# modelstreaming/ams

Measured on AMD Instinct MI355X. Metric: frames/sec student infer (DeeplabV3+MobileNetV2, 512x1024) + distill-steps/sec, higher is better.
Workload: dtype f32 (2xfp16 split products)

## Files before the change

ams_amd/csrc/k_pw_f16.hip:

```cpp
#include <type_traits>

#include "pw_common.hpp"
#include "split_bf16.hpp"

namespace ams {

__global__ void split_w_f16_kernel(const float* __restrict__ w, int64_t sk, int64_t sn, int K, int N, int Kp, unsigned short* __restrict__ hi,
                                   unsigned short* __restrict__ lo) {
    const int64_t i = blockIdx.x * (int64_t)blockDim.x + threadIdx.x;
    if (i >= (int64_t)N * Kp) return;
    const int n = (int)(i / Kp), k = (int)(i % Kp);
    const float v = k < K ? w[k * sk + n * sn] : 0.f;
    unsigned short h, l;
    split1_f16(v, h, l);
    hi[i] = h;
    lo[i] = l;
}

int launch_split_weights_f16(const float* w, int64_t sk, int64_t sn, int K, int N, int Kp, uint16_t* hi, uint16_t* lo, hipStream_t st) {
    const int64_t n = (int64_t)N * Kp;
    hipLaunchKernelGGL(split_w_f16_kernel, dim3(cdiv(n, 256)), dim3(256), 0, st, w, sk, sn, K, N, Kp, hi, lo);
    AMS_CHECK_LAUNCH();
    return AMS_OK;
}

__global__ void pack_h2i_kernel(const float* __restrict__ x, int64_t n8, u32x4* __restrict__ out) {
    const int64_t i = blockIdx.x * (int64_t)blockDim.x + threadIdx.x;
    if (i >= n8) return;
    const float4 u = ld4(x + 8 * i), v = ld4(x + 8 * i + 4);
    f16x8 h, l;
    split8_f16(u, v, h, l);
    out[2 * i] = __builtin_bit_cast(u32x4, h);
    out[2 * i + 1] = __builtin_bit_cast(u32x4, l);
}

int launch_pack_h2i(const float* x, int64_t M, int C, float* out, hipStream_t st) {
    AMS_REQUIRE(C % 8 == 0 && M > 0, "pack_h2i: C (%d) must be a multiple of 8", C);
    const int64_t n8 = M * (C / 8);
    hipLaunchKernelGGL(pack_h2i_kernel, dim3((unsigned)cdiv64(n8, 256)), dim3(256), 0, st, x, n8, reinterpret_cast<u32x4*>(out));
    AMS_CHECK_LAUNCH();
    return AMS_OK;
}

__device__ __forceinline__ f32x4 mma_f16(const u32x4& a, const u32x4& b, const f32x4& c) {
    return __builtin_amdgcn_mfma_f32_16x16x32_f16(__builtin_bit_cast(f16x8, a), __builtin_bit_cast(f16x8, b), c, 0, 0, 0);
}

constexpr int pwh_waves(int rm, int nt, int nw) { return nw >= 9 ? 3 : nw == 8 ? 2 : rm * nt > 12 ? 1 : rm * nt > 6 ? 2 : 3; }
constexpr int pwh_epw(int nw, int slab) { return nw * slab <= 60 * 1024 ? nw : nw % 5 == 0 && 5 * slab <= 60 * 1024 ? 5 : nw % 4 == 0 ? 4 : nw % 3 == 0 ? 3 : 1; }
constexpr bool pwh_dyn(int nw, int epi) { return nw >= 9 && epi != EPI_GENERIC; }

template <int RM, int NT, int EPI, int XP, int NW = 4, int D = 2, int ABL = 0, int XF = 0>
__global__ __launch_bounds__(64 * NW, pwh_waves(RM, NT, NW)) void pw_gemm_f16x3_l(PwArgs a, const unsigned short* __restrict__ w0, int64_t plane, int Kp,
                                                                                  int n_tiles_n, unsigned nblocks, unsigned n_full) {
    constexpr int NP = 2, NTH = 64 * NW;
    constexpr int PITCH = 32;
    constexpr int ROWS = 16 * NT;
    constexpr int NPIECE = NP * ROWS * 4;
    constexpr int NREG = (NPIECE + NTH - 1) / NTH;
    constexpr int SLAB = 16 * (16 * NT + 4) * 4;
    constexpr bool DYN = pwh_dyn(NW, EPI);
    constexpr int EPW = (EPI == EPI_GENERIC || DYN) ? NW : pwh_epw(NW, SLAB);
    static_assert(NW % EPW == 0, "epilogue rounds");
    static_assert(XF == 0 || (XP == 0 && EPI == EPI_PLAIN), "the operand transform runs on f32 operands with the plain epilogue");
    constexpr int W_BYTES = 2 * NP * ROWS * PITCH * 2, OUT_BYTES = EPI == EPI_GENERIC ? 16 : EPW * SLAB + (EPI == EPI_PLAIN && NW == 4 ? 4 * 16 * NT * 4 : 0);
    __shared__ __attribute__((aligned(16))) unsigned char smem_static[DYN ? 16 : (W_BYTES > OUT_BYTES ? W_BYTES : OUT_BYTES)];
    extern __shared__ __attribute__((aligned(16))) unsigned char smem_dyn[];
    unsigned char* smem = DYN ? smem_dyn : smem_static;
    typedef unsigned short (*WStage)[NP][ROWS * PITCH];
    WStage sW = reinterpret_cast<WStage>(smem);
    float* sOutAll = reinterpret_cast<float*>(smem);
    __shared__ __attribute__((aligned(16))) float sSc[16 * NT], sSh[16 * NT];
    constexpr int XVS = XF != 0 ? 1024 : 4;
    __shared__ __attribute__((aligned(16))) float sXv[XF == 1 ? 2 * XVS : 4];
    const bool half = blockIdx.x >= n_full;
    const unsigned lb = half ? xcd_remap(blockIdx.x - n_full, nblocks - n_full) : xcd_remap(blockIdx.x, n_full);
    const int tile_n = lb % n_tiles_n;
    const int64_t tile_m = lb / n_tiles_n;
    const int tid = threadIdx.x, wave = tid >> 6, lane = tid & 63, l15 = lane & 15, q = lane >> 4;
    const int n0 = tile_n * ROWS;
    const int nrg = half ? RM / 2 : RM;
    const int64_t m_base = half ? (int64_t)(n_full / n_tiles_n) * (16 * NW * RM) + tile_m * (8 * NW * RM) + wave * (8 * RM)
                                : tile_m * (16 * NW * RM) + wave * (16 * RM);
    const int K = a.K, n_stages = Kp / 32;
    const int n_iter = (n_stages + D - 1) / D * D;

    u32x4 wring[D][NREG];
    const unsigned short* wsrc[NREG];
    int wdst[NREG];
#pragma unroll
    for (int u = 0; u < NREG; ++u) {
        const int e = tid + u * NTH < NPIECE ? tid + u * NTH : NPIECE - 1;
        const int which = e / (ROWS * 4), r = e - which * (ROWS * 4), n = r >> 2, part = r & 3;
        int nn = n0 + n;
        if (nn > a.N - 1) nn = a.N - 1;
        wsrc[u] = w0 + which * plane + (int64_t)nn * Kp + part * 8;
        wdst[u] = which * (ROWS * PITCH) + n * PITCH + (part ^ (((n >> 3) & 1) << 1)) * 8;
    }
    auto load_stage = [&](int s, u32x4 (&wreg)[NREG]) {
        if (s > n_stages - 1) s = n_stages - 1;
#pragma unroll
        for (int u = 0; u < NREG; ++u) wreg[u] = *reinterpret_cast<const u32x4*>(wsrc[u] + s * 32);
    };
    auto store_stage = [&](int buf, const u32x4 (&wreg)[NREG]) {
        unsigned short* base = &sW[buf][0][0];
#pragma unroll
        for (int u = 0; u < NREG; ++u) *reinterpret_cast<u32x4*>(base + wdst[u]) = wreg[u];
    };
    const float* arow[RM];
#pragma unroll
    for (int r = 0; r < RM; ++r) {
        int64_t m = m_base + (r < nrg ? r : nrg - 1) * 16 + l15;
        if (m > a.M - 1) m = a.M - 1;
        arow[r] = a.x + m * (int64_t)a.ldx;
    }
    float4 abuf[D][RM][2];
    const float* aline[RM][2];
    if constexpr ((ABL & 16) != 0) {
#pragma unroll
        for (int r = 0; r < RM; ++r)
#pragma unroll
            for (int hf = 0; hf < 2; ++hf) {
                int64_t m = m_base + (r < nrg ? r : nrg - 1) * 16 + 8 * hf + (lane >> 3);
                if (m > a.M - 1) m = a.M - 1;
                aline[r][hf] = a.x + m * (int64_t)a.ldx + 4 * (lane & 7);
            }
    }
    auto load_a = [&](int s, float4 (&dst)[RM][2], auto Rc) {
        constexpr int R = decltype(Rc)::value;
        int koff = s * 32 + 8 * q;
        if (koff > K - 8) koff = K - 8;
        if constexpr ((ABL & 16) != 0) {
            int ks = s * 32;
            if (ks > K - 32) ks = K - 32;
#pragma unroll
            for (int r = 0; r < R; ++r) {
                dst[r][0] = ld4(aline[r][0] + ks);
                dst[r][1] = ld4(aline[r][1] + ks);
            }
            return;
        }
#pragma unroll
        for (int r = 0; r < R; ++r) {
            dst[r][0] = ld4(arow[r] + koff);
            dst[r][1] = ld4(arow[r] + koff + 4);
        }
    };
    typedef std::integral_constant<int, RM> RFull;
    typedef std::integral_constant<int, (RM >= 2 ? RM / 2 : RM)> RHalf;
    load_stage(0, wring[0]);
#pragma unroll
    for (int d = 0; d < D - 1; ++d) {
        if (d > 0) load_stage(d, wring[d]);
        load_a(d, abuf[d], RFull{});
    }
    f32x4 acc[RM][NT], accx[RM][NT];
#pragma unroll
    for (int r = 0; r < RM; ++r)
#pragma unroll
        for (int t = 0; t < NT; ++t) { acc[r][t] = (f32x4){0.f, 0.f, 0.f, 0.f}; accx[r][t] = (f32x4){0.f, 0.f, 0.f, 0.f}; }

    pw_stage_affine<NT>(a, sSc, sSh, n0, tid, NTH);
    if constexpr (XF != 0) {
        for (int e = tid; e < XVS; e += NTH) {
            const bool ok = e < K;
            sXv[e] = ok ? a.x_v0[e] : 0.f;
            sXv[XVS + e] = ok ? a.x_v1[e] : 0.f;
        }
    }
    store_stage(0, wring[0]);
    __syncthreads();
    auto main_loop = [&](auto Rc) {
        constexpr int R = decltype(Rc)::value;
        for (int s0 = 0; s0 < n_iter; s0 += D) {
#pragma unroll
            for (int d = 0; d < D; ++d) {
                const int s = s0 + d;
                if constexpr (!(ABL & 2)) load_stage(s + D - 1, wring[(d + D - 1) % D]);
                if constexpr (!(ABL & 1)) load_a(s + D - 1, abuf[(d + D - 1) % D], Rc);
                if (s < n_stages) {
                    u32x4 xh[RM], xl[RM];
                    float4 u0, u1, v0, v1;
                    if constexpr (XF != 0) {
                        int koff = s * 32 + 8 * q;
                        if (koff > K - 8) koff = K - 8;
                        u0 = ld4(sXv + koff); u1 = ld4(sXv + koff + 4); v0 = ld4(sXv + XVS + koff); v1 = ld4(sXv + XVS + koff + 4);
                    }
#pragma unroll
                    for (int r = 0; r < R; ++r) {
                        if constexpr (XF != 0) {
                            float4 y0 = muladd4_pk(abuf[d][r][0], u0, v0), y1 = muladd4_pk(abuf[d][r][1], u1, v1);
                            y0 = make_float4(apply_act(y0.x, a.x_act), apply_act(y0.y, a.x_act), apply_act(y0.z, a.x_act), apply_act(y0.w, a.x_act));
                            y1 = make_float4(apply_act(y1.x, a.x_act), apply_act(y1.y, a.x_act), apply_act(y1.z, a.x_act), apply_act(y1.w, a.x_act));
                            f16x8 h, l;
                            split8_f16(y0, y1, h, l);
                            xh[r] = __builtin_bit_cast(u32x4, h);
                            xl[r] = __builtin_bit_cast(u32x4, l);
                        } else if constexpr (XP) {
                            xh[r] = __builtin_bit_cast(u32x4, abuf[d][r][0]);
                            xl[r] = __builtin_bit_cast(u32x4, abuf[d][r][1]);
                        } else {
                            f16x8 h, l;
                            split8_f16(abuf[d][r][0], abuf[d][r][1], h, l);
                            xh[r] = __builtin_bit_cast(u32x4, h);
                            xl[r] = __builtin_bit_cast(u32x4, l);
                        }
                    }
                    const unsigned short* bw = &sW[s & 1][0][l15 * PITCH + 8 * (q ^ ((l15 >> 3) << 1))];
                    constexpr int TG = (ABL & 32) ? 5 : (NT >= 2 && RM <= 2) ? 2 : 1;
#pragma unroll
                    for (int t0 = 0; t0 < NT; t0 += TG) {
                        u32x4 qh[TG], ql[TG];
#pragma unroll
                        for (int g = 0; g < TG; ++g) {
                            if (t0 + g >= NT) continue;
                            qh[g] = *reinterpret_cast<const u32x4*>(bw + (t0 + g) * 16 * PITCH);
                            ql[g] = *reinterpret_cast<const u32x4*>(bw + (ROWS * PITCH) + (t0 + g) * 16 * PITCH);
                        }
#pragma unroll
                        for (int g = 0; g < TG; ++g)
#pragma unroll
                            for (int r = 0; r < R; ++r)
                                if (t0 + g < NT && !(ABL & 8)) { if constexpr ((ABL & 32) != 0) acc[r][t0 + g] = mma_f16(ql[g], xh[r], acc[r][t0 + g]); else accx[r][t0 + g] = mma_f16(ql[g], xh[r], accx[r][t0 + g]); }
#pragma unroll
                        for (int g = 0; g < TG; ++g)
#pragma unroll
                            for (int r = 0; r < R; ++r)
                                if (t0 + g < NT && !(ABL & 8)) { if constexpr ((ABL & 32) != 0) acc[r][t0 + g] = mma_f16(qh[g], xl[r], acc[r][t0 + g]); else accx[r][t0 + g] = mma_f16(qh[g], xl[r], accx[r][t0 + g]); }
#pragma unroll
                        for (int g = 0; g < TG; ++g)
#pragma unroll
                            for (int r = 0; r < R; ++r)
                                if (t0 + g < NT && !(ABL & 8)) acc[r][t0 + g] = mma_f16(qh[g], xh[r], acc[r][t0 + g]);
                        if constexpr ((ABL & 8) != 0) {
#pragma unroll
                            for (int g = 0; g < TG; ++g) if (t0 + g < NT) { acc[0][t0 + g][0] += __uint_as_float(qh[g][0] ^ ql[g][1]); acc[0][t0 + g][1] += __uint_as_float(xh[0][0] ^ xl[RM - 1][1]); }
                        }
                    }
                }
                if constexpr (!(ABL & 2)) store_stage((s + 1) & 1, wring[(d + 1) % D]);
                if constexpr (!(ABL & 4)) __syncthreads();
            }
        }
    };
    if (RM >= 2 && half) main_loop(RHalf{});
    else main_loop(RFull{});
#pragma unroll
    for (int r = 0; r < RM; ++r)
#pragma unroll
        for (int t = 0; t < NT; ++t) if constexpr (!(ABL & 32)) acc[r][t] = combine_f16(acc[r][t], accx[r][t]);
    const bool red = EPI == EPI_PLAIN && NW == 4 && a.red_mode != 0;
    float4 rs1[(EPI == EPI_PLAIN && NW == 4) ? NT : 1], rs2[(EPI == EPI_PLAIN && NW == 4) ? NT : 1];
    if constexpr (EPI == EPI_PLAIN && NW == 4) {
        if (red) {
            float* sRedVec = reinterpret_cast<float*>(smem) + 4 * 16 * (16 * NT + 4);
            pw_red_stage<NT>(a, sRedVec, n0, tid, NTH);
#pragma unroll
            for (int t = 0; t < NT; ++t) { rs1[t] = make_float4(0.f, 0.f, 0.f, 0.f); rs2[t] = rs1[t]; }
            __syncthreads();
            pw_red_rowgroups<RM, NT>(a, acc, m_base, n0, l15, q, sRedVec, rs1, rs2, nrg);
        }
    }
    if (EPI == EPI_GENERIC) pw_epilogue<RM, NT>(a, acc, m_base, n0, l15, q, sSc, sSh, nrg);
    else if constexpr (EPW == NW) pw_epilogue_t<RM, NT, EPI, true>(a, acc, m_base, n0, lane, sSc, sSh, sOutAll + wave * (16 * (16 * NT + 4)), nrg);
    else {
        for (int round = 0; round < NW / EPW; ++round) {
            if (wave / EPW == round) pw_epilogue_t<RM, NT, EPI, true>(a, acc, m_base, n0, lane, sSc, sSh, sOutAll + (wave % EPW) * (16 * (16 * NT + 4)), nrg);
            __syncthreads();
        }
    }
    if constexpr (EPI == EPI_PLAIN && NW == 4) {
        if (red) {
            __syncthreads();
            const int64_t row = half ? (int64_t)(n_full / n_tiles_n) + tile_m : tile_m;
            pw_red_finish<NT>(a, rs1, rs2, lane, wave, 4, reinterpret_cast<float*>(smem), row, n0, tid, NTH);
        }
    }
}

template <int RM, int NT, int EPI, int XP, int NW = 4, int D = 2, int ABL = 0, int XF = 0>
static int launch_pw_f16_d(const PwArgs& a, const uint16_t* w, int64_t plane, int Kp, hipStream_t st) {
    const int n_tiles_n = cdiv(a.N, 16 * NT);
    int per_cu = 1, cus = 256;
    constexpr size_t kSlab = 16 * (16 * NT + 4) * 4, kW = (size_t)2 * 2 * 16 * NT * 32 * 2;
    const size_t dyn = pwh_dyn(NW, EPI) ? (NW * kSlab > kW ? NW * kSlab : kW) : 0;
    if (dyn) RUN_RC(func_allow_lds((const void*)pw_gemm_f16x3_l<RM, NT, EPI, XP, NW, D, ABL, XF>, dyn));
    RUN_RC(func_blocks_per_cu((const void*)pw_gemm_f16x3_l<RM, NT, EPI, XP, NW, D, ABL, XF>, 64 * NW, dyn, &per_cu));
    RUN_RC(device_cus(&cus));
    int64_t half_strips = 0;
    const int64_t full_strips = pw_plan_tail(a.M, RM, n_tiles_n, per_cu * cus, &half_strips, 16 * NW * RM);
    const int64_t n_full = full_strips * n_tiles_n;
    const int64_t nblocks = n_full + half_strips * n_tiles_n;
    PwArgs b = a;
    if (b.red_mode) {
        if (EPI == EPI_PLAIN && NW == 4 && b.red_mode == 1 && pw_red_ok(b, nblocks / n_tiles_n)) { if (b.red_rows_out) *b.red_rows_out = (int)(nblocks / n_tiles_n); }
        else { b.red_mode = 0; if (b.red_rows_out) *b.red_rows_out = 0; }
    }
    static const std::string nm = "pw_gemm_f16x3_l<" + std::to_string(RM) + ", " + std::to_string(NT) + ", " + std::to_string(EPI) + ", " + std::to_string(XP) + ", " +
                                  std::to_string(NW) + ", " + std::to_string(D) + ", " + std::to_string(ABL) + ", " + std::to_string(XF) + ">";
    note_kernel(nm.c_str());
    hipLaunchKernelGGL((pw_gemm_f16x3_l<RM, NT, EPI, XP, NW, D, ABL, XF>), dim3((unsigned)nblocks), dim3(64 * NW), dyn, st, b, w, plane, Kp, n_tiles_n,
                       (unsigned)nblocks, (unsigned)n_full);
    AMS_CHECK_LAUNCH();
    return AMS_OK;
}

template <int RM, int NT>
static int launch_pw_f16(const PwArgs& a, const uint16_t* w, int64_t plane, int Kp, hipStream_t st) {
    const int epi = pw_pick_epi(a);
    if (a.x_mode == 1) return launch_pw_f16_d<RM, NT, EPI_PLAIN, 0, 4, 2, 0, 1>(a, w, plane, Kp, st);
#ifdef AMS_MEASURE
    if constexpr (RM == 2 && NT == 5) {
        const int abl = knobs().pwh_abl;
        if (abl && a.x_fmt == 1) {
#define PWH_A(A_) if (abl == A_) return launch_pw_f16_d<RM, NT, EPI_PLAIN, 1, 4, 2, A_>(a, w, plane, Kp, st);
            PWH_A(1) PWH_A(2) PWH_A(3) PWH_A(4) PWH_A(6) PWH_A(7) PWH_A(8) PWH_A(9) PWH_A(10) PWH_A(11) PWH_A(15)
#undef PWH_A
        }
    }
#endif
    if constexpr (NT == 10 && RM <= 2) {
        int nw = knobs().pwh_nw, dd = knobs().pwh_d;
        if (!knobs().pwh_set && RM == 1) { nw = a.N <= 160 ? 10 : 12; dd = 3; }
#ifdef AMS_MEASURE
        if constexpr (RM == 1) {
            const int abl = knobs().pwh_abl;
            if (abl && a.x_fmt == 1 && nw == 12 && dd == 3) {
#define PWH_A(A_) if (abl == A_) return launch_pw_f16_d<RM, NT, EPI_PLAIN, 1, 12, 3, A_>(a, w, plane, Kp, st);
                PWH_A(1) PWH_A(2) PWH_A(3) PWH_A(8) PWH_A(9) PWH_A(10) PWH_A(11) PWH_A(16) PWH_A(18) PWH_A(24) PWH_A(26) PWH_A(32) PWH_A(35) PWH_A(48) PWH_A(15) PWH_A(4)
#undef PWH_A
            }
        }
#endif
        if (a.x_fmt == 1 && (epi == EPI_PLAIN || epi == EPI_RES) && (nw > 4 || dd > 2)) {
#define PWH_V(NW_, D_) if (nw == NW_ && dd == D_) return epi == EPI_PLAIN ? launch_pw_f16_d<RM, NT, EPI_PLAIN, 1, NW_, D_>(a, w, plane, Kp, st) : launch_pw_f16_d<RM, NT, EPI_RES, 1, NW_, D_>(a, w, plane, Kp, st);
            PWH_V(8, 2) PWH_V(12, 2) PWH_V(8, 3) PWH_V(12, 3) PWH_V(10, 3)
#undef PWH_V
        }
    }
    if constexpr (RM == 2 && (NT == 5 || NT == 4)) {
        const int nw = knobs().pwh_nw, dd = knobs().pwh_d;
        if (a.x_fmt == 1 && (epi == EPI_PLAIN || epi == EPI_RES) && (nw > 4 || dd > 2)) {
#define PWH_V(NW_, D_) if (nw == NW_ && dd == D_) return epi == EPI_PLAIN ? launch_pw_f16_d<RM, NT, EPI_PLAIN, 1, NW_, D_>(a, w, plane, Kp, st) : launch_pw_f16_d<RM, NT, EPI_RES, 1, NW_, D_>(a, w, plane, Kp, st);
            PWH_V(4, 3) PWH_V(4, 4) PWH_V(8, 2) PWH_V(8, 3) PWH_V(12, 2) PWH_V(12, 3)
#undef PWH_V
        }
    }
    if (a.x_fmt == 1) {
        switch (epi) {
            case EPI_PLAIN: return launch_pw_f16_d<RM, NT, EPI_PLAIN, 1>(a, w, plane, Kp, st);
            case EPI_RES: return launch_pw_f16_d<RM, NT, EPI_RES, 1>(a, w, plane, Kp, st);
            case EPI_BIAS: return launch_pw_f16_d<RM, NT, EPI_BIAS, 1>(a, w, plane, Kp, st);
            default: return launch_pw_f16_d<RM, NT, EPI_GENERIC, 1>(a, w, plane, Kp, st);
        }
    }
    switch (epi) {
        case EPI_PLAIN: return launch_pw_f16_d<RM, NT, EPI_PLAIN, 0>(a, w, plane, Kp, st);
        case EPI_RES: return launch_pw_f16_d<RM, NT, EPI_RES, 0>(a, w, plane, Kp, st);
        case EPI_BIAS: return launch_pw_f16_d<RM, NT, EPI_BIAS, 0>(a, w, plane, Kp, st);
        default: return launch_pw_f16_d<RM, NT, EPI_GENERIC, 0>(a, w, plane, Kp, st);
    }
}

bool pointwise_f16_applies(const PwArgs& a) {
    if (!(a.M > 0 && a.K >= 32 && a.K % 8 == 0 && a.ldx % 4 == 0 && a.Kw == a.K && (a.x_fmt == 0 || a.ldx == a.K))) return false;
    if (a.red_mode > 1) return false;
    if (a.x_mode == 0) return true;
    return a.x_mode == 1 && a.x_fmt == 0 && a.x_v0 && a.x_v1 && a.K <= 1024 && pw_pick_epi(a) == EPI_PLAIN;
}

int launch_pointwise_split_f16(const PwArgs& a, const uint16_t* whi, int64_t plane, int Kp, hipStream_t st) {
    if (a.red_rows_out) *a.red_rows_out = 0;
    AMS_REQUIRE(pointwise_f16_applies(a) && Kp % 32 == 0 && Kp >= a.K, "pointwise_split_f16: bad problem (M %lld K %d ldx %d)", (long long)a.M, a.K, a.ldx);
    int rm, nt;
    pw_pick_tile(a.M, a.N, &rm, &nt);
    if (rm == 2) {
        if (a.N == 96 || a.N == 960) nt = 6;
        else if (a.N == 320) nt = 5;
    }
    if (a.M <= 2400 && rm == 1 && a.N % 32 == 0 && a.N >= 64) nt = 2;
    const int epi0 = pw_pick_epi(a);
    if (a.x_fmt == 1 && a.N % 160 == 0 && a.M >= 16384 && (epi0 == EPI_PLAIN || epi0 == EPI_RES)) { rm = 1; nt = 10; }
    if (knobs().pwx_rm > 0) { rm = knobs().pwx_rm; nt = knobs().pwx_nt; }
#define PW_H(RM_, NT_) if (rm == RM_ && nt == NT_) return launch_pw_f16<RM_, NT_>(a, whi, plane, Kp, st);
    PW_H(2, 6) PW_H(2, 5) PW_H(2, 4) PW_H(2, 3) PW_H(2, 2) PW_H(2, 1)
    PW_H(1, 6) PW_H(1, 5) PW_H(1, 4) PW_H(1, 3) PW_H(1, 2) PW_H(1, 1)
    PW_H(2, 8) PW_H(2, 10) PW_H(1, 10) PW_H(4, 4) PW_H(4, 3)
#undef PW_H
    set_error("pointwise_split_f16: no tile configuration");
    return AMS_E_INVALID;
}

}
```

ams_amd/csrc/kernels.hpp:

```cpp
#pragma once
#include <vector>

#include "common.hpp"

struct ams_comm;

namespace ams {

struct ConvLayer;
struct BlockCall;

int func_allow_lds(const void* fn, size_t lds);
int func_blocks_per_cu(const void* fn, int threads, size_t lds, int* per_cu);
int device_cus(int* cus);
bool launch_table_needs_attr(int device, const void* fn, size_t lds);
struct Knobs {
    int blk_th = 0, blk_tw = 0;
    int fb_walk = -1;
    int fb_abl = 0;
    int xwr_timed = 0;
    int blk_timed = 0;
    int blk_hp = -1;
    char pw_force = 0; int pw_rm = 0, pw_nt = 0;
    int pw_percu = 0;
    bool pwx_no_tail = false;
    int pwx_rm = 0, pwx_nt = 0;
    int xwr_abl = 0;
    int pwh_abl = 0;
    bool pwh_set = false; int pwh_nw = 4, pwh_d = 2;
    bool xds_set = false; int xds[6] = {0, 0, 0, 0, 0, 0};
    bool xwr_set = false; int xwr[5] = {0, 0, 0, 0, 0};
    bool wg6_eight_waves = false;
    int wg6_split_cap = 0;
    int event_flags = -1;
    unsigned side_cu_mask = 0;
};
const Knobs& knobs();
int blk_phase_cycles(unsigned long long* h);
int xwr_phase_cycles(unsigned long long* h);
int xds_phase_cycles(unsigned long long* h);
int create_side_stream(hipStream_t* out);
int create_sync_event(hipEvent_t* out);

int comm_allreduce(ams_comm* c, void* p, size_t n, int dtype, hipStream_t st);

struct PwArgs {
    const float* x;
    int64_t M;
    int K;
    int Kw;
    int ldx;
    const float* w;
    int64_t w_sk, w_sn;
    int N;
    const float* img_bias;
    int64_t rows_per_img;
    const float* scale;
    const float* shift;
    int act;
    const float* res;
    int ldr;
    float* y;
    int ldy;
    uint16_t* ysplit;
    int64_t ysplit_plane;
    int ysplit_np;
    int ysplit_fmt;
    int y_skip_f32;
    int x_fmt;
    int red_mode;
    const float* red_center;
    const float* red_z; const float* red_scale; const float* red_shift; const float* red_mean; const float* red_rstd;
    int red_act;
    float* red_part;
    size_t red_part_floats;
    int* red_rows_out;
    const float* red_res; int red_ldr;
    int x_mode; int x_act;
    const float* x_v0; const float* x_v1; const float* x_v2; const float* x2;
    float* x_tmp;
};
static inline PwArgs pw_args(const float* x, int64_t M, int K, int ldx, const float* w, int N, float* y, int ldy) {
    PwArgs a;
    memset(&a, 0, sizeof(a));
    a.x = x; a.M = M; a.K = K; a.Kw = K; a.ldx = ldx; a.w = w; a.w_sk = N; a.w_sn = 1; a.N = N;
    a.rows_per_img = 1; a.act = AMS_ACT_NONE; a.y = y; a.ldy = ldy;
    return a;
}
int launch_pointwise(const PwArgs& a, hipStream_t st);
int pointwise_materialize_x(const PwArgs& a, PwArgs* b, hipStream_t st);
bool pointwise_stream_applies(const PwArgs& a);
bool pointwise_transforms_on_load(const PwArgs& a);
bool pointwise_split3_transforms_on_load(const PwArgs& a);

int launch_split_weights(const float* w, int64_t sk, int64_t sn, int K, int N, int Kp, uint16_t* hi, uint16_t* lo, hipStream_t st);
int launch_pointwise_split(const PwArgs& a, const uint16_t* whi, const uint16_t* wlo, int Kp, hipStream_t st);
int launch_split_weights3(const float* w, int64_t sk, int64_t sn, int K, int N, int Kp, uint16_t* hi, uint16_t* mid, uint16_t* lo,
                          hipStream_t st);
int launch_pointwise_split3(const PwArgs& a, const uint16_t* whi, const uint16_t* wmid, const uint16_t* wlo, int Kp, hipStream_t st);
struct SplitJob { const float* w; int64_t sk, sn; int K, N, Kp; uint16_t* p0; int64_t plane; int64_t first_block; int f16; };
int launch_split_batch(const SplitJob* jobs_dev, int njobs, int64_t total_blocks, hipStream_t st, int write_f16);
int launch_pointwise_split1(const PwArgs& a, const uint16_t* whi, int Kp, hipStream_t st);
int launch_split_weights_f16(const float* w, int64_t sk, int64_t sn, int K, int N, int Kp, uint16_t* hi, uint16_t* lo, hipStream_t st);
bool pointwise_f16_applies(const PwArgs& a);
int launch_pointwise_split_f16(const PwArgs& a, const uint16_t* whi, int64_t plane, int Kp, hipStream_t st);
int launch_pack_h2i(const float* x, int64_t M, int C, float* out, hipStream_t st);
bool pointwise_split_writes_parts(const PwArgs& a);
bool head_chain_supported(int KA, int NA, int KB, int NB, int KC, int NC);
int launch_head_chain(const float* x, int64_t M, int KA, const ConvLayer& A, const ConvLayer& B, const ConvLayer& C, const float* img_bias,
                      int64_t rows_per_img, int NC, float* y, hipStream_t st);

struct WgArgs {
    const float* x;  int ldx;  int K;
    const float* dy; int ldy;  int N;
    int64_t M;
    float* dw;
    float* scratch; size_t scratch_floats;
    int allow_split;
    int x_mode = 0, x_act = 0; const float* x_v0 = nullptr; const float* x_v1 = nullptr;
    int dy_mode = 0; const float* dy_v0 = nullptr; const float* dy_v1 = nullptr; const float* dy_v2 = nullptr; const float* dy2 = nullptr;
};
bool dw_project_supported(int C, int N, int stride, int rate);
int launch_dw_project(const BlockCall& c, hipStream_t st);
bool pointwise_wgrad_x6_applies(int64_t M, int K, int N, int ldx, int ldy);
int wgrad_x6_splits(int64_t M, int K, int N);
int launch_pointwise_wgrad_x6(const WgArgs& a, int splits, hipStream_t st);
size_t pointwise_wgrad_scratch(int64_t M, int K, int N);
int launch_pointwise_wgrad(const WgArgs& a, hipStream_t st);

struct FirstBlockPlan {
    int Ho, Wo, pt, pl;
    int tiles_y, tiles_x;
    int ity0, itx0, niy, nix;
    int interior_tiles, interior_grid;
    int border_tiles, border_grid;
    int border_walks;
};
int first_block_plan(int dtype, int B, int H, int W, bool h16, const int* occupancy, FirstBlockPlan* plan);
int launch_first_block(const BlockCall& c, hipStream_t st, FirstBlockPlan* plan_out = nullptr);

int launch_resize_u8(const uint8_t* src, int Hs, int Ws, int C, int mode, int swap_rb, uint8_t* dst, int H, int W, hipStream_t st);

int launch_stem(const void* frames, int dtype, int B, int H, int W, const float* w, int cout, const float* scale,
                const float* shift, int act, float pixel_scale, float* y, hipStream_t st);
int launch_stem_im2col(const void* frames, int dtype, int B, int H, int W, float pixel_scale, float* out, hipStream_t st);
int launch_depthwise(const float* x, int B, int H, int W, int C, const float* w, int stride, int rate,
                     const float* scale, const float* shift, int act, float* y, hipStream_t st);
int launch_depthwise_dgrad(const float* dy, int B, int H, int W, int C, const float* w, int stride, int rate,
                           float* dx, hipStream_t st);
size_t depthwise_fwd_bn_scratch(int B, int H, int W, int C, int rate);
int launch_depthwise_fwd_bn(const float* ze, int B, int H, int W, int C, const float* w, int rate, const float* scale, const float* shift, int act,
                            const float* center, float* zd, float* scratch, int* rows_out, hipStream_t st);
size_t depthwise_dgrad_bn_scratch(int B, int H, int W, int C);
int launch_depthwise_dgrad_bn(const float* dy, int B, int H, int W, int C, const float* w, int rate, const float* z, const float* scale,
                              const float* shift, int act, const float* mean, const float* rstd, float* out, float* scratch, int* rows_out,
                              hipStream_t st);
size_t depthwise_dgrad_bn2_scratch(int B, int H, int W, int C, int rate);
int launch_depthwise_dgrad_bn2(const float* dy, const float* zd, const float* cA, const float* cB, const float* cC, int B, int H, int W, int C,
                               const float* w, int rate, const float* ze, const float* scale, const float* shift, int act, const float* mean,
                               const float* rstd, float* out, float* scratch, int* rows_out, hipStream_t st);
size_t depthwise_fwd_bn2_scratch(int B, int H, int W, int C, int rate);
int launch_depthwise_fwd_bn2(const float* ze, int B, int H, int W, int C, const float* w, int rate, const float* scale, const float* shift, int act,
                             const float* center, float* zd, float* scratch, int* rows_out, hipStream_t st);
size_t depthwise_wgrad_scratch(int B, int H, int W, int C, int stride, int rate);
int launch_depthwise_wgrad(const float* x, const float* dy, int B, int H, int W, int C, int stride, int rate,
                           float* dw, float* scratch, size_t scratch_floats, hipStream_t st);

bool expand_dw_supported(int Cin, int Cexp, int stride, int rate);
size_t expand_dw_stats_scratch(int B, int H, int W, int Cexp, int stride);
int launch_expand_dw(const BlockCall& c, hipStream_t st, const float* stats_center = nullptr, float* stats_part = nullptr, int* stats_rows = nullptr);

bool xdw_train_supported(int Cin, int Cexp, int stride, int rate);
size_t xdw_train_scratch(int B, int H, int W, int Cin, int Cexp);
int xdw_train_blocks(int B, int H, int W, int Cexp);
int launch_xdw_fwd_stats(const float* x, int B, int H, int W, int Cin, const float* w_exp, int Cexp, const float* center, float* scratch,
                         int* rows_out, int64_t* stride_out, hipStream_t st);
int launch_xdw_bwd_reduce(const float* x, int B, int H, int W, int Cin, const float* w_exp, int Cexp, const float* sc_e, const float* sh_e,
                          const float* mean_e, const float* rstd_e, int act_e, const float* w_dw, int stride, const float* dz_d, float* scratch,
                          int* rows_out, int64_t* stride_out, hipStream_t st);
size_t xdw_stem_scratch(int B, int fH, int fW);
int launch_xdw_bwd_reduce_stem(const void* frames, int dtype, int B, int fH, int fW, float pixel_scale, const float* w_stem, const float* sc_e,
                               const float* sh_e, const float* mean_e, const float* rstd_e, int act_e, const float* w_dw, const float* dz_d,
                               float* scratch, int* rows_out, int64_t* stride_out, hipStream_t st);
int launch_xdw_bwd_dx(const float* x, int B, int H, int W, int Cin, const float* w_exp, int Cexp, const float* sc_e, const float* sh_e,
                      int act_e, const float* w_dw, int stride, const float* dz_d, const float* cA, const float* cB, const float* cC,
                      const float* res, float* dx, hipStream_t st, const float* red_z = nullptr, const float* red_mean = nullptr,
                      const float* red_rstd = nullptr, float* red_part = nullptr, int* red_rows_out = nullptr);
int launch_xdw_dwe(const float* G1, const float* xx_g0, int Cin, int Cexp, const float* w_exp, const float* cA, const float* cB, const float* cC,
                   float* dw, hipStream_t st);

int xx_stats_blocks(int64_t M);
size_t xx_stats_scratch_doubles(int64_t M, int Cin);
int launch_xx_gram(const float* x, int64_t M, int Cin, double* scratch, double* xx64, float* xx32, hipStream_t st);
int launch_expand_stats(const double* xx64, int Cin, const float* w_exp, int Cexp, double n, const float* center, const float* gamma,
                        const float* beta, float eps, float one_minus_decay, float* moving_mean, float* moving_var, float* scale, float* shift,
                        float* save_mean, float* save_rstd, double* sums, hipStream_t st);

bool block_fused_supported(int Cin, int Cexp, int Cout, int stride, int rate, bool residual);
int launch_block_fused(const BlockCall& c, hipStream_t st);
int launch_first_block_tiles(const BlockCall& c, hipStream_t st);
int launch_block_pack(const float* sc_e, const float* sh_e, const float* sc_d, const float* sh_d, const float* w_dw, int Cexp, float* out, hipStream_t st);

constexpr int AMS_NP_F16 = 4;
bool expand_dw_stream_supported(int Cin, int Cexp, int stride, int rate);
int launch_expand_dw_stream(const BlockCall& c, hipStream_t st);

int launch_expand_dw_wreg(const BlockCall& c, hipStream_t st);


size_t image_colsum_scratch(int B, int C);
int launch_global_mean(const float* x, int B, int64_t HW, int C, float* y, float* scratch, hipStream_t st);
int launch_image_colsum(const float* x, int B, int64_t HW, int C, int ldx, float* out, float* scratch, hipStream_t st);

size_t colstats_scratch(int64_t M, int C);
int launch_colstats(const float* z, int64_t M, int C, const float* center, double* sums , float* scratch,
                    hipStream_t st);
int launch_colstats_f64(const float* z, int64_t M, int C, const float* center, double* sums , hipStream_t st);
int launch_bn_finalize(const double* sums, double n, int C, const float* center, const float* gamma, const float* beta,
                       float eps, float one_minus_decay, float* moving_mean, float* moving_var, float* scale,
                       float* shift, float* save_mean, float* save_rstd, hipStream_t st);
int launch_bn_fold(const float* gamma, const float* beta, const float* mean, const float* var, float eps, int C,
                   float* scale, float* shift, hipStream_t st);
int launch_bn_act(const float* z, int64_t M, int C, const float* scale, const float* shift, int act, const float* res,
                  float* a, hipStream_t st);
int launch_bn_bwd_reduce(const float* da, const float* z, int64_t M, int C, const float* scale, const float* shift,
                         int act, const float* mean, const float* rstd, double* sums, float* scratch, hipStream_t st);
int launch_bn_bwd_coef(const double* sums, double n, int C, const float* gamma, const float* mean, const float* rstd,
                       float* coefA, float* coefB, float* coefC, float* dgamma, float* dbeta, hipStream_t st);
int launch_bn_param_grads(const double* sums, int C, float* dgamma, float* dbeta, hipStream_t st);
int launch_colstats_bn(const float* z, int64_t M, int C, const float* center, double* sums, float* scratch, double n,
                       const float* gamma, const float* beta, float eps, float one_minus_decay, float* moving_mean,
                       float* moving_var, float* scale, float* shift, float* save_mean, float* save_rstd, hipStream_t st);
int launch_bn_bwd_reduce_coef(const float* da, const float* z, int64_t M, int C, const float* scale, const float* shift, int act,
                              const float* mean, const float* rstd, double* sums, float* scratch, double n, const float* gamma,
                              float* coefA, float* coefB, float* coefC, float* dgamma, float* dbeta, hipStream_t st);
int launch_bn_bwd_apply(const float* da, const float* z, int64_t M, int C, const float* scale, const float* shift, int act,
                        const float* coefA, const float* coefB, const float* coefC, float* dz, hipStream_t st);
int launch_colsum(const float* x, int64_t M, int C, int ldx, float* out, float* scratch, hipStream_t st);
int launch_adam(float* p, const float* g, float* m, float* v, const uint8_t* mask, int64_t n, float lr_t, float b1,
                float b2, float eps, hipStream_t st);
struct ReduceJobs {
    static constexpr int kMax = 32;
    int n = 0;
    const float* part[kMax]; float* out[kMax]; int splits[kMax]; int64_t count[kMax]; int64_t stride[kMax]; int first_block[kMax];
    bool add(const float* p, int splits_, int64_t count_, float* o, int64_t stride_) {
        if (n >= kMax) return false;
        part[n] = p; splits[n] = splits_; count[n] = count_; out[n] = o; stride[n] = stride_ > 0 ? stride_ : count_; ++n;
        return true;
    }
};
int launch_reduce_batch(ReduceJobs& jobs, hipStream_t st);
int launch_reduce_splits(const float* part, int splits, int64_t n, float* out, hipStream_t st, int64_t stride = 0);
int launch_bn_fwd_finalize_partials(const float* part, int rows, int64_t row_stride, int C, double* sums, double n, const float* center,
                                    const float* gamma, const float* beta, float eps, float one_minus_decay, float* moving_mean,
                                    float* moving_var, float* scale, float* shift, float* save_mean, float* save_rstd, hipStream_t st);
int launch_bn_bwd_finalize_partials(const float* part, int rows, int64_t row_stride, int C, double* sums, double n, const float* gamma,
                                    const float* mean, const float* rstd, float* coefA, float* coefB, float* coefC, float* dgamma,
                                    float* dbeta, hipStream_t st);
int launch_partials_to_sums(const float* part, int rows, int64_t row_stride, int C, double* sums, hipStream_t st);
int launch_fill(float* p, int64_t n, float v, hipStream_t st);
int launch_round_bf16(float* p, int64_t n, hipStream_t st);
int launch_copy(float* dst, const float* src, int64_t n, hipStream_t st);
size_t pack_fp16_scratch(int64_t n);
int launch_pack_fp16(const float* p, const uint8_t* mask, int64_t n, uint16_t* out, int64_t* n_out, int64_t* counts, hipStream_t st);
int64_t delta_segments(int64_t mask_bytes);
int launch_apply_delta(const uint8_t* payload, int64_t payload_bytes, const ams_delta_var* vars_dev, int n_vars, int64_t mask_bytes,
                       float* params, int64_t n_params, float* stats, int64_t n_stats, int64_t* counts, int64_t* n_applied, int32_t* status,
                       hipStream_t st);
size_t select_scratch();
int launch_select_changed(const float* after, const float* before, int64_t n, int64_t k, ams_select_result* result, int64_t* scratch,
                          hipStream_t st);
int launch_select_apply(float* params, const float* before, int64_t n, float cut, uint8_t* mask, int64_t* n_kept, hipStream_t st);
int64_t encode_segments(int64_t mask_bytes);
int launch_encode_delta(const uint8_t* mask, const int64_t* table_dev, int n_vars, int64_t mask_bytes, const float* params, const float* stats,
                        int64_t* work, uint8_t* payload, int64_t cap, int64_t* payload_bytes, hipStream_t st);

struct HeadCall;
struct LossObjective;
int launch_upsample_argmax(const HeadCall& c, int32_t* labels, int64_t* conf, double* loss, hipStream_t st, int per_frame = 0,
                           int labels_u8 = 0 );
int launch_ce_grad(const HeadCall& c, const double* loss_and_count, float* dlogits, int ldd, hipStream_t st, float empty_val = 0.f);
bool ce_loss_grad_supported(int w, int W);
size_t ce_loss_grad_scratch(int B, int h, int w, int K);
int launch_ce_loss_grad(const HeadCall& c, const LossObjective& o, double* loss, float* scratch, hipStream_t st);
int launch_ce_combine(const HeadCall& c, const double* loss_and_count, const float* scratch, float* dlogits, int ldd, hipStream_t st,
                      float empty_val = 0.f);
struct WeightRange { const float* w; int64_t n; };
int weights_beyond(const std::vector<WeightRange>& jobs, float limit, float low, int* flags_dev , int* over_host,
                   hipStream_t st);
int launch_l2_regularizer(const float* p, float* g, const uint8_t* mask, int64_t n, int n_vars, float coef, double* part_scratch ,
                          double* loss, hipStream_t st);
int launch_cross_confusion(const uint8_t* a, const uint8_t* b, int64_t n, const int32_t* lut ,
                           int K, int64_t* conf, hipStream_t st);

int confidence_stats_len();
int launch_upsample_confidence(const HeadCall& c, uint8_t* conf_u8, float* conf_f32, int64_t* stats, hipStream_t st);

int soft_metric_stats_len(int K);
int launch_upsample_soft_metric(const HeadCall& c, const LossObjective& o, int64_t* stats, float* p_f32, float* ce_f32, hipStream_t st);

struct MiningBuffers { float* keys = nullptr; uint8_t* labels = nullptr; uint32_t* hist = nullptr; ams_mining_result* result = nullptr; };
size_t loss_mining_scratch(int B, int H, int W);
MiningBuffers loss_mining_buffers(void* scratch, int B, int H, int W);
int mining_top_k_check(const char* who, float top_k);
int launch_mining_keys(const HeadCall& c, const LossObjective& o, float top_k, const MiningBuffers& m, hipStream_t st);
int launch_mining_select(int64_t n, float top_k, const MiningBuffers& m, hipStream_t st);
int launch_mining_relabel(const uint8_t* labels, int64_t n, const MiningBuffers& m, hipStream_t st);
int launch_loss_mining(const HeadCall& c, const LossObjective& o, float top_k, const MiningBuffers& m, hipStream_t st);

int launch_replay_gather(const uint8_t* frame_slots, int64_t frame_stride, const uint8_t* label_slots, int64_t label_stride, int capacity, int Hs,
                         int Ws, const ams_replay_sample* samples_dev, const ams_replay_sample* samples_host, int B, int H, int W,
                         uint8_t* frames_out, uint8_t* labels_out, hipStream_t st);
int launch_replay_gather_rows(const float* slots, int64_t slot_stride, int capacity, int th, int tw, int C, const ams_replay_sample* samples_dev,
                              const ams_replay_sample* samples_host, int B, float* out, hipStream_t st);
int launch_replay_gather_logits(const float* slots, int64_t slot_stride, int capacity, int Hs, int Ws, int C, const ams_replay_sample* samples_dev,
                                const ams_replay_sample* samples_host, int B, int H, int W, float* out, hipStream_t st);
int launch_replay_gather_logits_lowres(const float* slots, int64_t slot_stride, int capacity, int lh, int lw, int C, int Hs, int Ws,
                                       const ams_replay_sample* samples_dev, const ams_replay_sample* samples_host, int B, int H, int W, float* out,
                                       hipStream_t st);
int launch_replay_pack_logits(const float* in, int th, int tw, int NC, const int32_t* idx_host, int K, float* out, hipStream_t st);
int launch_teacher_labels_from_logits(const float* logits, int64_t slot_stride, int n, int lh, int lw, int NC, int Hs, int Ws, uint8_t* out,
                                      int64_t out_stride, hipStream_t st);
int launch_cross_confusion_pairs(const uint8_t* label_slots, int64_t label_stride, int capacity, int64_t n, const int32_t* pairs_dev,
                                 const int32_t* pairs_host, int n_pairs, const int32_t* lut , int K, int64_t* conf,
                                 hipStream_t st);

int launch_render_views(const uint8_t* frames, const void* student, int student_dtype, const uint8_t* teacher, int B, int H, int W, int K,
                        const uint8_t* tables, const ams_render_out* out, hipStream_t st);

}
```

ams_amd/csrc/runtime.hip:

```cpp
#include <stdlib.h>

#include <map>
#include <mutex>
#include <tuple>

#include "kernels.hpp"

namespace ams {

namespace {
std::mutex g_mu;
std::map<std::pair<int, const void*>, size_t> g_attr;
std::map<std::tuple<int, const void*, int, size_t>, int> g_occ;
std::map<int, int> g_cus;
}

bool launch_table_needs_attr(int device, const void* fn, size_t lds) {
    std::lock_guard<std::mutex> lk(g_mu);
    size_t& have = g_attr[{device, fn}];
    if (lds <= have) return false;
    have = lds;
    return true;
}

int func_allow_lds(const void* fn, size_t lds) {
    if (lds <= 64 * 1024) return AMS_OK;
    int dev = 0;
    AMS_CHECK_HIP(hipGetDevice(&dev));
    std::lock_guard<std::mutex> lk(g_mu);
    auto it = g_attr.find({dev, fn});
    if (it != g_attr.end() && lds <= it->second) return AMS_OK;
    const hipError_t e = hipFuncSetAttribute(fn, hipFuncAttributeMaxDynamicSharedMemorySize, (int)lds);
    if (e != hipSuccess) {
        set_error("hipFuncSetAttribute(dynamic LDS %zu) -> %s", lds, hipGetErrorString(e));
        return AMS_E_HIP;
    }
    g_attr[{dev, fn}] = lds;
    return AMS_OK;
}

int func_blocks_per_cu(const void* fn, int threads, size_t lds, int* per_cu) {
    int dev = 0;
    AMS_CHECK_HIP(hipGetDevice(&dev));
    {
        std::lock_guard<std::mutex> lk(g_mu);
        auto it = g_occ.find({dev, fn, threads, lds});
        if (it != g_occ.end()) { *per_cu = it->second; return AMS_OK; }
    }
    int nb = 0;
    if (hipOccupancyMaxActiveBlocksPerMultiprocessor(&nb, fn, threads, lds) != hipSuccess || nb < 1) nb = 1;
    std::lock_guard<std::mutex> lk(g_mu);
    g_occ[{dev, fn, threads, lds}] = nb;
    *per_cu = nb;
    return AMS_OK;
}

int device_cus(int* cus) {
    int dev = 0;
    AMS_CHECK_HIP(hipGetDevice(&dev));
    {
        std::lock_guard<std::mutex> lk(g_mu);
        auto it = g_cus.find(dev);
        if (it != g_cus.end()) { *cus = it->second; return AMS_OK; }
    }
    int n = 0;
    AMS_CHECK_HIP(hipDeviceGetAttribute(&n, hipDeviceAttributeMultiprocessorCount, dev));
    std::lock_guard<std::mutex> lk(g_mu);
    g_cus[dev] = n;
    *cus = n;
    return AMS_OK;
}

static Knobs read_knobs() {
        Knobs v;
        if (const char* e = getenv("AMS_BLK_TILE")) sscanf(e, "%dx%d", &v.blk_th, &v.blk_tw);
        if (const char* e = getenv("AMS_BLK_HP")) v.blk_hp = atoi(e);
        if (const char* e = getenv("AMS_FB_WALK")) v.fb_walk = atoi(e);
        if (const char* e = getenv("AMS_BLK_TIMED")) v.blk_timed = atoi(e);
        if (const char* e = getenv("AMS_XWR_TIMED")) v.xwr_timed = atoi(e);
        if (const char* e = getenv("AMS_PW_FORCE")) sscanf(e, "%c,%d,%d", &v.pw_force, &v.pw_rm, &v.pw_nt);
        if (const char* e = getenv("AMS_PW_PERCU")) v.pw_percu = atoi(e);
        v.pwx_no_tail = getenv("AMS_PWX_NO_TAIL") != nullptr;
#ifdef AMS_MEASURE
        if (const char* e = getenv("AMS_FB_ABL")) v.fb_abl = atoi(e);
        if (const char* e = getenv("AMS_PWH_ABL")) v.pwh_abl = atoi(e);
        if (const char* e = getenv("AMS_XWR_ABL")) v.xwr_abl = atoi(e);
#else
        for (const char* name : {"AMS_FB_ABL", "AMS_PWH_ABL", "AMS_XWR_ABL"})
            if (const char* e = getenv(name))
                if (atoi(e) != 0) fprintf(stderr, "libams_hip: %s=%s ignored — ablated kernels exist only in libams_hip_measure.so (make -C ams_amd/csrc measure)\n", name, e);
#endif
        if (const char* e = getenv("AMS_PWH_VARIANT")) { v.pwh_set = true; sscanf(e, "%d,%d", &v.pwh_nw, &v.pwh_d); }
        if (const char* e = getenv("AMS_PWX_FORCE")) sscanf(e, "%d,%d", &v.pwx_rm, &v.pwx_nt);
        if (const char* e = getenv("AMS_XDS_FORCE")) { v.xds_set = true; sscanf(e, "%d,%d,%d,%d,%d,%d", &v.xds[0], &v.xds[1], &v.xds[2], &v.xds[3], &v.xds[4], &v.xds[5]); }
        if (const char* e = getenv("AMS_XWR_FORCE")) { v.xwr_set = true; sscanf(e, "%d,%d,%d,%d,%d", &v.xwr[0], &v.xwr[1], &v.xwr[2], &v.xwr[3], &v.xwr[4]); }
        if (const char* e = getenv("AMS_WG6_SPLITS")) v.wg6_split_cap = atoi(e);
        v.wg6_eight_waves = getenv("AMS_WG6_EIGHT_WAVES") != nullptr;
        if (const char* e = getenv("AMS_SIDE_CU_MASK")) v.side_cu_mask = (unsigned)strtoul(e, nullptr, 16);
        if (const char* e = getenv("AMS_EVENT_FLAGS")) v.event_flags = (int)strtoul(e, nullptr, 16);
        return v;
}
static Knobs& knobs_storage() {
    static Knobs k = read_knobs();
    return k;
}
const Knobs& knobs() { return knobs_storage(); }

int create_sync_event(hipEvent_t* out) {
    const unsigned flags = knobs().event_flags >= 0 ? (unsigned)knobs().event_flags : (unsigned)hipEventDisableTiming;
    AMS_CHECK_HIP(hipEventCreateWithFlags(out, flags));
    return AMS_OK;
}

int create_side_stream(hipStream_t* out) {
    if (knobs().side_cu_mask) {
        uint32_t mask[8];
        for (int i = 0; i < 8; ++i) mask[i] = knobs().side_cu_mask;
        AMS_CHECK_HIP(hipExtStreamCreateWithCUMask(out, 8, mask));
        return AMS_OK;
    }
    AMS_CHECK_HIP(hipStreamCreateWithFlags(out, hipStreamNonBlocking));
    return AMS_OK;
}

}

extern "C" int ams_debug_reload_knobs(void) {
    ams::knobs_storage() = ams::read_knobs();
    return AMS_OK;
}

extern "C" int ams_debug_launch_table_needs_attr(int32_t device, uint64_t kernel_key, size_t lds) {
    return ams::launch_table_needs_attr(device, (const void*)(uintptr_t)kernel_key, lds) ? 1 : 0;
}
```

Before: 12950.

## Add three-stage LDS weight ring with fragment read-ahead for wide H2I pointwise GEMM

Adds an FA template mode to the f16x3 pointwise GEMM. FA=2 uses three LDS weight stages fed from a three-deep register ring, and double-buffers the MFMA weight fragments so the next group's LDS reads are issued before the current MFMAs. Scheduling barriers keep that ordering in place. It is enabled by default for RM=1, NT=10 layers with N<=160 and K<=576, and aims to hide LDS read latency behind the matrix ops. The cost is more LDS per block and more registers, which may lower occupancy.

```diff
diff --git a/ams_amd/csrc/k_pw_f16.hip b/ams_amd/csrc/k_pw_f16.hip
--- a/ams_amd/csrc/k_pw_f16.hip
+++ b/ams_amd/csrc/k_pw_f16.hip
@@ -50,7 +50,7 @@
 constexpr int pwh_epw(int nw, int slab) { return nw * slab <= 60 * 1024 ? nw : nw % 5 == 0 && 5 * slab <= 60 * 1024 ? 5 : nw % 4 == 0 ? 4 : nw % 3 == 0 ? 3 : 1; }
 constexpr bool pwh_dyn(int nw, int epi) { return nw >= 9 && epi != EPI_GENERIC; }
 
-template <int RM, int NT, int EPI, int XP, int NW = 4, int D = 2, int ABL = 0, int XF = 0>
+template <int RM, int NT, int EPI, int XP, int NW = 4, int D = 2, int ABL = 0, int XF = 0, int FA = 0>
 __global__ __launch_bounds__(64 * NW, pwh_waves(RM, NT, NW)) void pw_gemm_f16x3_l(PwArgs a, const unsigned short* __restrict__ w0, int64_t plane, int Kp,
                                                                                   int n_tiles_n, unsigned nblocks, unsigned n_full) {
     constexpr int NP = 2, NTH = 64 * NW;
@@ -58,12 +58,17 @@
     constexpr int ROWS = 16 * NT;
     constexpr int NPIECE = NP * ROWS * 4;
     constexpr int NREG = (NPIECE + NTH - 1) / NTH;
+    constexpr int LS = FA == 2 ? 3 : 2;
+    constexpr int NG = NT / 2;
+    constexpr int U = FA == 2 ? 6 : D;
+    static_assert(FA == 0 || (pwh_dyn(NW, EPI) && XP == 1 && XF == 0 && RM == 1 && NT % 2 == 0 && (ABL & ~11) == 0), "fragment read-ahead: wide H2I blocks");
+    static_assert(FA != 2 || D == 3, "three LDS stages take their weights from a register ring of three");
     constexpr int SLAB = 16 * (16 * NT + 4) * 4;
     constexpr bool DYN = pwh_dyn(NW, EPI);
     constexpr int EPW = (EPI == EPI_GENERIC || DYN) ? NW : pwh_epw(NW, SLAB);
     static_assert(NW % EPW == 0, "epilogue rounds");
     static_assert(XF == 0 || (XP == 0 && EPI == EPI_PLAIN), "the operand transform runs on f32 operands with the plain epilogue");
-    constexpr int W_BYTES = 2 * NP * ROWS * PITCH * 2, OUT_BYTES = EPI == EPI_GENERIC ? 16 : EPW * SLAB + (EPI == EPI_PLAIN && NW == 4 ? 4 * 16 * NT * 4 : 0);
+    constexpr int W_BYTES = LS * NP * ROWS * PITCH * 2, OUT_BYTES = EPI == EPI_GENERIC ? 16 : EPW * SLAB + (EPI == EPI_PLAIN && NW == 4 ? 4 * 16 * NT * 4 : 0);
     __shared__ __attribute__((aligned(16))) unsigned char smem_static[DYN ? 16 : (W_BYTES > OUT_BYTES ? W_BYTES : OUT_BYTES)];
     extern __shared__ __attribute__((aligned(16))) unsigned char smem_dyn[];
     unsigned char* smem = DYN ? smem_dyn : smem_static;
@@ -83,7 +88,7 @@
     const int64_t m_base = half ? (int64_t)(n_full / n_tiles_n) * (16 * NW * RM) + tile_m * (8 * NW * RM) + wave * (8 * RM)
                                 : tile_m * (16 * NW * RM) + wave * (16 * RM);
     const int K = a.K, n_stages = Kp / 32;
-    const int n_iter = (n_stages + D - 1) / D * D;
+    const int n_iter = (n_stages + U - 1) / U * U;
 
     u32x4 wring[D][NREG];
     const unsigned short* wsrc[NREG];
@@ -169,14 +174,30 @@
         }
     }
     store_stage(0, wring[0]);
+    if constexpr (FA == 2) {
+        load_stage(2, wring[2]);
+        store_stage(1, wring[1]);
+    }
     __syncthreads();
+    const int frag_off = l15 * PITCH + 8 * (q ^ ((l15 >> 3) << 1));
+    u32x4 fqh[2][2], fql[2][2];
+    auto read_frags = [&](int buf, int t0, u32x4 (&h)[2], u32x4 (&l)[2]) {
+        const unsigned short* b = &sW[buf][0][frag_off];
+#pragma unroll
+        for (int g = 0; g < 2; ++g) {
+            h[g] = *reinterpret_cast<const u32x4*>(b + (t0 + g) * 16 * PITCH);
+            l[g] = *reinterpret_cast<const u32x4*>(b + (ROWS * PITCH) + (t0 + g) * 16 * PITCH);
+        }
+    };
+    if constexpr (FA == 2) read_frags(0, 0, fqh[0], fql[0]);
     auto main_loop = [&](auto Rc) {
         constexpr int R = decltype(Rc)::value;
-        for (int s0 = 0; s0 < n_iter; s0 += D) {
-#pragma unroll
-            for (int d = 0; d < D; ++d) {
+        for (int s0 = 0; s0 < n_iter; s0 += U) {
+#pragma unroll
+            for (int d = 0; d < U; ++d) {
                 const int s = s0 + d;
-                if constexpr (!(ABL & 2)) load_stage(s + D - 1, wring[(d + D - 1) % D]);
+                if constexpr (FA == 2) { if constexpr (!(ABL & 2)) load_stage(s + D, wring[d % D]); }
+                else if constexpr (!(ABL & 2)) load_stage(s + D - 1, wring[(d + D - 1) % D]);
                 if constexpr (!(ABL & 1)) load_a(s + D - 1, abuf[(d + D - 1) % D], Rc);
                 if (s < n_stages) {
                     u32x4 xh[RM], xl[RM];
@@ -189,7 +210,7 @@
 #pragma unroll
                     for (int r = 0; r < R; ++r) {
                         if constexpr (XF != 0) {
-                            float4 y0 = muladd4_pk(abuf[d][r][0], u0, v0), y1 = muladd4_pk(abuf[d][r][1], u1, v1);
+                            float4 y0 = muladd4_pk(abuf[d % D][r][0], u0, v0), y1 = muladd4_pk(abuf[d % D][r][1], u1, v1);
                             y0 = make_float4(apply_act(y0.x, a.x_act), apply_act(y0.y, a.x_act), apply_act(y0.z, a.x_act), apply_act(y0.w, a.x_act));
                             y1 = make_float4(apply_act(y1.x, a.x_act), apply_act(y1.y, a.x_act), apply_act(y1.z, a.x_act), apply_act(y1.w, a.x_act));
                             f16x8 h, l;
@@ -197,15 +218,39 @@
                             xh[r] = __builtin_bit_cast(u32x4, h);
                             xl[r] = __builtin_bit_cast(u32x4, l);
                         } else if constexpr (XP) {
-                            xh[r] = __builtin_bit_cast(u32x4, abuf[d][r][0]);
-                            xl[r] = __builtin_bit_cast(u32x4, abuf[d][r][1]);
+                            xh[r] = __builtin_bit_cast(u32x4, abuf[d % D][r][0]);
+                            xl[r] = __builtin_bit_cast(u32x4, abuf[d % D][r][1]);
                         } else {
                             f16x8 h, l;
-                            split8_f16(abuf[d][r][0], abuf[d][r][1], h, l);
+                            split8_f16(abuf[d % D][r][0], abuf[d % D][r][1], h, l);
                             xh[r] = __builtin_bit_cast(u32x4, h);
                             xl[r] = __builtin_bit_cast(u32x4, l);
                         }
                     }
+                    if constexpr (FA != 0) {
+                        const int buf = FA == 2 ? d % LS : (s & 1);
+                        const int p0 = FA == 2 ? (d * NG) & 1 : 0;
+                        if constexpr (FA == 1) read_frags(buf, 0, fqh[p0], fql[p0]);
+#pragma unroll
+                        for (int gi = 0; gi < NG; ++gi) {
+                            const int cur = (p0 + gi) & 1, t0 = 2 * gi;
+                            if (gi + 1 < NG) read_frags(buf, t0 + 2, fqh[cur ^ 1], fql[cur ^ 1]);
+                            else if constexpr (FA == 2) read_frags((d + 1) % LS, 0, fqh[cur ^ 1], fql[cur ^ 1]);
+                            __builtin_amdgcn_sched_barrier(0);
+                            if constexpr (!(ABL & 8)) {
+#pragma unroll
+                                for (int g = 0; g < 2; ++g) accx[0][t0 + g] = mma_f16(fql[cur][g], xh[0], accx[0][t0 + g]);
+#pragma unroll
+                                for (int g = 0; g < 2; ++g) accx[0][t0 + g] = mma_f16(fqh[cur][g], xl[0], accx[0][t0 + g]);
+#pragma unroll
+                                for (int g = 0; g < 2; ++g) acc[0][t0 + g] = mma_f16(fqh[cur][g], xh[0], acc[0][t0 + g]);
+                            } else {
+#pragma unroll
+                                for (int g = 0; g < 2; ++g) { acc[0][t0 + g][0] += __uint_as_float(fqh[cur][g][0] ^ fql[cur][g][1]); acc[0][t0 + g][1] += __uint_as_float(xh[0][0] ^ xl[0][1]); }
+                            }
+                            __builtin_amdgcn_sched_barrier(0);
+                        }
+                    } else {
                     const unsigned short* bw = &sW[s & 1][0][l15 * PITCH + 8 * (q ^ ((l15 >> 3) << 1))];
                     constexpr int TG = (ABL & 32) ? 5 : (NT >= 2 && RM <= 2) ? 2 : 1;
 #pragma unroll
@@ -237,8 +282,10 @@
                             for (int g = 0; g < TG; ++g) if (t0 + g < NT) { acc[0][t0 + g][0] += __uint_as_float(qh[g][0] ^ ql[g][1]); acc[0][t0 + g][1] += __uint_as_float(xh[0][0] ^ xl[RM - 1][1]); }
                         }
                     }
+                    }
                 }
-                if constexpr (!(ABL & 2)) store_stage((s + 1) & 1, wring[(d + 1) % D]);
+                if constexpr (FA == 2) { if constexpr (!(ABL & 2)) store_stage((d + 2) % LS, wring[(d + 2) % D]); }
+                else if constexpr (!(ABL & 2)) store_stage((s + 1) & 1, wring[(d + 1) % D]);
                 if constexpr (!(ABL & 4)) __syncthreads();
             }
         }
@@ -278,14 +325,14 @@
     }
 }
 
-template <int RM, int NT, int EPI, int XP, int NW = 4, int D = 2, int ABL = 0, int XF = 0>
+template <int RM, int NT, int EPI, int XP, int NW = 4, int D = 2, int ABL = 0, int XF = 0, int FA = 0>
 static int launch_pw_f16_d(const PwArgs& a, const uint16_t* w, int64_t plane, int Kp, hipStream_t st) {
     const int n_tiles_n = cdiv(a.N, 16 * NT);
     int per_cu = 1, cus = 256;
-    constexpr size_t kSlab = 16 * (16 * NT + 4) * 4, kW = (size_t)2 * 2 * 16 * NT * 32 * 2;
+    constexpr size_t kSlab = 16 * (16 * NT + 4) * 4, kW = (size_t)(FA == 2 ? 3 : 2) * 2 * 16 * NT * 32 * 2;
     const size_t dyn = pwh_dyn(NW, EPI) ? (NW * kSlab > kW ? NW * kSlab : kW) : 0;
-    if (dyn) RUN_RC(func_allow_lds((const void*)pw_gemm_f16x3_l<RM, NT, EPI, XP, NW, D, ABL, XF>, dyn));
-    RUN_RC(func_blocks_per_cu((const void*)pw_gemm_f16x3_l<RM, NT, EPI, XP, NW, D, ABL, XF>, 64 * NW, dyn, &per_cu));
+    if (dyn) RUN_RC(func_allow_lds((const void*)pw_gemm_f16x3_l<RM, NT, EPI, XP, NW, D, ABL, XF, FA>, dyn));
+    RUN_RC(func_blocks_per_cu((const void*)pw_gemm_f16x3_l<RM, NT, EPI, XP, NW, D, ABL, XF, FA>, 64 * NW, dyn, &per_cu));
     RUN_RC(device_cus(&cus));
     int64_t half_strips = 0;
     const int64_t full_strips = pw_plan_tail(a.M, RM, n_tiles_n, per_cu * cus, &half_strips, 16 * NW * RM);
@@ -297,9 +344,9 @@
         else { b.red_mode = 0; if (b.red_rows_out) *b.red_rows_out = 0; }
     }
     static const std::string nm = "pw_gemm_f16x3_l<" + std::to_string(RM) + ", " + std::to_string(NT) + ", " + std::to_string(EPI) + ", " + std::to_string(XP) + ", " +
-                                  std::to_string(NW) + ", " + std::to_string(D) + ", " + std::to_string(ABL) + ", " + std::to_string(XF) + ">";
+                                  std::to_string(NW) + ", " + std::to_string(D) + ", " + std::to_string(ABL) + ", " + std::to_string(XF) + ", " + std::to_string(FA) + ">";
     note_kernel(nm.c_str());
-    hipLaunchKernelGGL((pw_gemm_f16x3_l<RM, NT, EPI, XP, NW, D, ABL, XF>), dim3((unsigned)nblocks), dim3(64 * NW), dyn, st, b, w, plane, Kp, n_tiles_n,
+    hipLaunchKernelGGL((pw_gemm_f16x3_l<RM, NT, EPI, XP, NW, D, ABL, XF, FA>), dim3((unsigned)nblocks), dim3(64 * NW), dyn, st, b, w, plane, Kp, n_tiles_n,
                        (unsigned)nblocks, (unsigned)n_full);
     AMS_CHECK_LAUNCH();
     return AMS_OK;
@@ -321,10 +368,16 @@
 #endif
     if constexpr (NT == 10 && RM <= 2) {
         int nw = knobs().pwh_nw, dd = knobs().pwh_d;
-        if (!knobs().pwh_set && RM == 1) { nw = a.N <= 160 ? 10 : 12; dd = 3; }
+        int fa = knobs().pwh_fa;
+        if (!knobs().pwh_set && RM == 1) { nw = a.N <= 160 ? 10 : 12; dd = 3; fa = a.N <= 160 && a.K <= 576 ? 2 : 0; }
 #ifdef AMS_MEASURE
         if constexpr (RM == 1) {
             const int abl = knobs().pwh_abl;
+            if (abl && a.x_fmt == 1 && nw == 12 && dd == 3 && fa == 2) {
+#define PWH_A(A_) if (abl == A_) return launch_pw_f16_d<RM, NT, EPI_PLAIN, 1, 12, 3, A_, 0, 2>(a, w, plane, Kp, st);
+                PWH_A(1) PWH_A(2) PWH_A(3) PWH_A(8) PWH_A(9) PWH_A(10) PWH_A(11)
+#undef PWH_A
+            }
             if (abl && a.x_fmt == 1 && nw == 12 && dd == 3) {
 #define PWH_A(A_) if (abl == A_) return launch_pw_f16_d<RM, NT, EPI_PLAIN, 1, 12, 3, A_>(a, w, plane, Kp, st);
                 PWH_A(1) PWH_A(2) PWH_A(3) PWH_A(8) PWH_A(9) PWH_A(10) PWH_A(11) PWH_A(16) PWH_A(18) PWH_A(24) PWH_A(26) PWH_A(32) PWH_A(35) PWH_A(48) PWH_A(15) PWH_A(4)
@@ -333,6 +386,14 @@
         }
 #endif
         if (a.x_fmt == 1 && (epi == EPI_PLAIN || epi == EPI_RES) && (nw > 4 || dd > 2)) {
+            if constexpr (RM == 1) {
+#define PWH_F(NW_, D_, FA_) if (nw == NW_ && dd == D_ && fa == FA_) return epi == EPI_PLAIN ? launch_pw_f16_d<RM, NT, EPI_PLAIN, 1, NW_, D_, 0, 0, FA_>(a, w, plane, Kp, st) : launch_pw_f16_d<RM, NT, EPI_RES, 1, NW_, D_, 0, 0, FA_>(a, w, plane, Kp, st);
+                PWH_F(10, 3, 2) PWH_F(12, 3, 2)
+#ifdef AMS_MEASURE
+                PWH_F(10, 2, 1) PWH_F(12, 2, 1)
+#endif
+#undef PWH_F
+            }
 #define PWH_V(NW_, D_) if (nw == NW_ && dd == D_) return epi == EPI_PLAIN ? launch_pw_f16_d<RM, NT, EPI_PLAIN, 1, NW_, D_>(a, w, plane, Kp, st) : launch_pw_f16_d<RM, NT, EPI_RES, 1, NW_, D_>(a, w, plane, Kp, st);
             PWH_V(8, 2) PWH_V(12, 2) PWH_V(8, 3) PWH_V(12, 3) PWH_V(10, 3)
 #undef PWH_V
diff --git a/ams_amd/csrc/kernels.hpp b/ams_amd/csrc/kernels.hpp
--- a/ams_amd/csrc/kernels.hpp
+++ b/ams_amd/csrc/kernels.hpp
@@ -27,7 +27,7 @@
     int pwx_rm = 0, pwx_nt = 0;
     int xwr_abl = 0;
     int pwh_abl = 0;
-    bool pwh_set = false; int pwh_nw = 4, pwh_d = 2;
+    bool pwh_set = false; int pwh_nw = 4, pwh_d = 2, pwh_fa = 0;
     bool xds_set = false; int xds[6] = {0, 0, 0, 0, 0, 0};
     bool xwr_set = false; int xwr[5] = {0, 0, 0, 0, 0};
     bool wg6_eight_waves = false;
diff --git a/ams_amd/csrc/runtime.hip b/ams_amd/csrc/runtime.hip
--- a/ams_amd/csrc/runtime.hip
+++ b/ams_amd/csrc/runtime.hip
@@ -90,7 +90,7 @@
             if (const char* e = getenv(name))
                 if (atoi(e) != 0) fprintf(stderr, "libams_hip: %s=%s ignored — ablated kernels exist only in libams_hip_measure.so (make -C ams_amd/csrc measure)\n", name, e);
 #endif
-        if (const char* e = getenv("AMS_PWH_VARIANT")) { v.pwh_set = true; sscanf(e, "%d,%d", &v.pwh_nw, &v.pwh_d); }
+        if (const char* e = getenv("AMS_PWH_VARIANT")) { v.pwh_set = true; sscanf(e, "%d,%d,%d", &v.pwh_nw, &v.pwh_d, &v.pwh_fa); }
         if (const char* e = getenv("AMS_PWX_FORCE")) sscanf(e, "%d,%d", &v.pwx_rm, &v.pwx_nt);
         if (const char* e = getenv("AMS_XDS_FORCE")) { v.xds_set = true; sscanf(e, "%d,%d,%d,%d,%d,%d", &v.xds[0], &v.xds[1], &v.xds[2], &v.xds[3], &v.xds[4], &v.xds[5]); }
         if (const char* e = getenv("AMS_XWR_FORCE")) { v.xwr_set = true; sscanf(e, "%d,%d,%d,%d,%d", &v.xwr[0], &v.xwr[1], &v.xwr[2], &v.xwr[3], &v.xwr[4]); }
```

Measured after the change: 12910. No clear change (-0.4%).
